# privefl/bigsnpr

Hardware: NVIDIA H100
Metric: genotypes/sec in bed_prodVec (higher is better)
Workload: dtype f64

## Files before the change

### bigsnpr_b200/csrc/bsg_pmv.cu

```cuda
#include <algorithm>
#include <math.h>
#include <stdio.h>
#include <stdlib.h>
#include <string.h>

#include <cub/device/device_scan.cuh>

#include "bsg_internal.cuh"
#include "bsg_pmv_shared.cuh"

namespace bsg {
namespace pmv {

constexpr int SEG = 128;
constexpr int CODES = 512;
constexpr int DIG = 4096;
constexpr int STAGES = 6;
constexpr int STAGE_BYTES = 2 * DIG;
constexpr int SMEM_BYTES = STAGES * STAGE_BYTES + 128;
constexpr int MAX_CHUNKS_PER_ITEM = 512;

struct Args {
  const uint8_t *P;
  int64_t stride;
  const int *lines;
  int nlines;
  int nlines_pad;
  int nchunks;
  int chunks_per_split;
  int ksplit;
  const uint8_t *dig1;
  const uint8_t *dig2;
  const uint8_t *na_flags;
  int use_na;
  long long *part;
};

struct Slot {
  uint4 alo, ahi, blo, bhi;
};

__device__ __forceinline__ void slot_load(Slot &s, const uint8_t *pa, const uint8_t *pb, int64_t off) {
  s.alo = ldg_stream(pa + off);
  s.ahi = ldg_stream(pa + off + 64);
  s.blo = ldg_stream(pb + off);
  s.bhi = ldg_stream(pb + off + 64);
}

template <int MODE>
__device__ __forceinline__ uint32_t plane2(uint32_t x) {
  return MODE == 3 ? (x >> 1) : (x & (x >> 1));
}

template <int MODE, bool PRE>
__device__ __forceinline__ void chunk_mma(const Slot &t0, const Slot &t1, uint32_t dig_addr, int (&acc1)[2][4],
                                          int (&acc16)[2][4], int (&accn1)[2][4], int (&accn16)[2][4]) {
  const uint32_t wA0[8] = {t0.alo.x, t0.alo.y, t0.alo.z, t0.alo.w, t0.ahi.x, t0.ahi.y, t0.ahi.z, t0.ahi.w};
  const uint32_t wB0[8] = {t0.blo.x, t0.blo.y, t0.blo.z, t0.blo.w, t0.bhi.x, t0.bhi.y, t0.bhi.z, t0.bhi.w};
  const uint32_t wA1[8] = {t1.alo.x, t1.alo.y, t1.alo.z, t1.alo.w, t1.ahi.x, t1.ahi.y, t1.ahi.z, t1.ahi.w};
  const uint32_t wB1[8] = {t1.blo.x, t1.blo.y, t1.blo.z, t1.blo.w, t1.bhi.x, t1.bhi.y, t1.bhi.z, t1.bhi.w};
  uint4 dpre[8];
  if (PRE) {
#pragma unroll
    for (int w = 0; w < 8; w++) dpre[w] = lds128(dig_addr + w * 512);
  }
#pragma unroll
  for (int w = 0; w < 8; w++) {
    const uint4 d = PRE ? dpre[w] : lds128(dig_addr + w * 512);
    const uint32_t a0 = wA0[w], b0 = wB0[w], a1 = wA1[w], b1 = wB1[w];
    const uint32_t a0t = a0 >> 2, b0t = b0 >> 2, a1t = a1 >> 2, b1t = b1 >> 2;
    mma_u8s8(acc1[0], a0 & 0x03030303u, b0 & 0x03030303u, a0t & 0x03030303u, b0t & 0x03030303u, d.x, d.y);
    mma_u8s8(acc1[1], a1 & 0x03030303u, b1 & 0x03030303u, a1t & 0x03030303u, b1t & 0x03030303u, d.x, d.y);
    mma_u8s8(acc16[0], a0 & 0x30303030u, b0 & 0x30303030u, a0t & 0x30303030u, b0t & 0x30303030u, d.z, d.w);
    mma_u8s8(acc16[1], a1 & 0x30303030u, b1 & 0x30303030u, a1t & 0x30303030u, b1t & 0x30303030u, d.z, d.w);
    if (MODE != 0) {
      uint4 dn = d;
      if (MODE >= 2) dn = lds128(dig_addr + DIG + w * 512);
      const uint32_t a0n = plane2<MODE>(a0), b0n = plane2<MODE>(b0), a0nt = plane2<MODE>(a0t), b0nt = plane2<MODE>(b0t);
      const uint32_t a1n = plane2<MODE>(a1), b1n = plane2<MODE>(b1), a1nt = plane2<MODE>(a1t), b1nt = plane2<MODE>(b1t);
      mma_u8s8(accn1[0], a0n & 0x01010101u, b0n & 0x01010101u, a0nt & 0x01010101u, b0nt & 0x01010101u, dn.x, dn.y);
      mma_u8s8(accn1[1], a1n & 0x01010101u, b1n & 0x01010101u, a1nt & 0x01010101u, b1nt & 0x01010101u, dn.x, dn.y);
      mma_u8s8(accn16[0], a0n & 0x10101010u, b0n & 0x10101010u, a0nt & 0x10101010u, b0nt & 0x10101010u, dn.z, dn.w);
      mma_u8s8(accn16[1], a1n & 0x10101010u, b1n & 0x10101010u, a1nt & 0x10101010u, b1nt & 0x10101010u, dn.z, dn.w);
    }
  }
}

template <int MODE>
__device__ __forceinline__ void tile_mma(const Slot &sl, const uint4 (&b1)[8], uint32_t dig2_addr, int (&acc1)[4],
                                         int (&acc16)[4], int (&accn1)[4], int (&accn16)[4]) {
  const uint32_t wA[8] = {sl.alo.x, sl.alo.y, sl.alo.z, sl.alo.w, sl.ahi.x, sl.ahi.y, sl.ahi.z, sl.ahi.w};
  const uint32_t wB[8] = {sl.blo.x, sl.blo.y, sl.blo.z, sl.blo.w, sl.bhi.x, sl.bhi.y, sl.bhi.z, sl.bhi.w};
#pragma unroll
  for (int w = 0; w < 8; w++) {
    const uint32_t a = wA[w], bq = wB[w];
    const uint32_t at = a >> 2, bt = bq >> 2;
    mma_u8s8(acc1, a & 0x03030303u, bq & 0x03030303u, at & 0x03030303u, bt & 0x03030303u, b1[w].x, b1[w].y);
    mma_u8s8(acc16, a & 0x30303030u, bq & 0x30303030u, at & 0x30303030u, bt & 0x30303030u, b1[w].z, b1[w].w);
    if (MODE != 0) {
      uint4 d = b1[w];
      if (MODE >= 2) d = lds128(dig2_addr + w * 512);
      const uint32_t an = plane2<MODE>(a), bn = plane2<MODE>(bq);
      const uint32_t ant = plane2<MODE>(at), bnt = plane2<MODE>(bt);
      mma_u8s8(accn1, an & 0x01010101u, bn & 0x01010101u, ant & 0x01010101u, bnt & 0x01010101u, d.x, d.y);
      mma_u8s8(accn16, an & 0x10101010u, bn & 0x10101010u, ant & 0x10101010u, bnt & 0x10101010u, d.z, d.w);
    }
  }
}

template <int MODE, int CW, int R, int STRUCT>
__global__ void __launch_bounds__((CW + 1) * 32, 1) k_pmv(const Args a) {
  constexpr int GROUP = CW * 32;
  extern __shared__ __align__(128) uint8_t smem[];
  const int warp = threadIdx.x >> 5, lane = threadIdx.x & 31;
  const uint32_t smem_base = smem_u32(smem);
  const uint32_t bar_base = smem_base + STAGES * STAGE_BYTES;

  if (threadIdx.x == 0) {
    for (int s = 0; s < STAGES; s++) {
      mbar_init(bar_base + 8 * s, 1);
      mbar_init(bar_base + 8 * (STAGES + s), CW);
    }
    asm volatile("fence.mbarrier_init.release.cluster;" ::: "memory");
  }
  __syncthreads();

  const int ngroups = a.nlines_pad / GROUP;
  const int nitems = ngroups * a.ksplit;
  constexpr bool two_dig = MODE >= 2;
  const uint32_t stage_tx = DIG + (two_dig ? DIG : 0);

  int stage = 0;
  uint32_t phase = 0;

  if (warp == CW) {
    if (lane == 0) {
      for (int item = blockIdx.x; item < nitems; item += gridDim.x) {
        const int group = item / a.ksplit, ks = item - group * a.ksplit;
        const int c0 = ks * a.chunks_per_split;
        const int c1 = min(a.nchunks, c0 + a.chunks_per_split);
        for (int c = c0; c < c1; c++) {
          const uint32_t full = bar_base + 8 * stage, empty = bar_base + 8 * (STAGES + stage);
          mbar_wait(empty, phase ^ 1);
          mbar_expect_tx(full, stage_tx);
          const uint32_t dst = smem_base + stage * STAGE_BYTES;
          bulk_g2s(dst, a.dig1 + (int64_t)c * DIG, DIG, full);
          if (two_dig) bulk_g2s(dst + DIG, a.dig2 + (int64_t)c * DIG, DIG, full);
          if (++stage == STAGES) {
            stage = 0;
            phase ^= 1;
          }
        }
      }
    }
  } else {
    const int g = lane >> 2, q = lane & 3;
    for (int item = blockIdx.x; item < nitems; item += gridDim.x) {
      const int group = item / a.ksplit, ks = item - group * a.ksplit;
      const int c0 = ks * a.chunks_per_split;
      const int c1 = min(a.nchunks, c0 + a.chunks_per_split);
      const uint8_t *pA[2], *pB[2];
#pragma unroll
      for (int u = 0; u < 2; u++) {
        int la = min(group * GROUP + warp * 32 + u * 16 + g, a.nlines - 1);
        int lb = min(group * GROUP + warp * 32 + u * 16 + g + 8, a.nlines - 1);
        const int pa = a.lines ? a.lines[la] : la, pb = a.lines ? a.lines[lb] : lb;
        pA[u] = a.P + (int64_t)pa * a.stride + 16 * q;
        pB[u] = a.P + (int64_t)pb * a.stride + 16 * q;
      }
      bool tile_na = false;
      if (MODE == 3) {
        tile_na = true;
      } else if (MODE != 0) {
        if (a.na_flags) {
          int l = min(group * GROUP + warp * 32 + lane, a.nlines - 1);
          const int phys = a.lines ? a.lines[l] : l;
          tile_na = __any_sync(0xffffffffu, a.na_flags[phys] != 0);
        } else {
          tile_na = true;
        }
      }
      int acc1[2][4], acc16[2][4], accn1[2][4], accn16[2][4];
#pragma unroll
      for (int u = 0; u < 2; u++)
#pragma unroll
        for (int k = 0; k < 4; k++) acc1[u][k] = acc16[u][k] = accn1[u][k] = accn16[u][k] = 0;

      Slot ring[R][2];
#pragma unroll
      for (int k = 0; k < R; k++) {
        ring[k][0] = ring[k][1] =
            Slot{make_uint4(0, 0, 0, 0), make_uint4(0, 0, 0, 0), make_uint4(0, 0, 0, 0), make_uint4(0, 0, 0, 0)};
        if (c0 + k < c1) {
          slot_load(ring[k][0], pA[0], pB[0], (int64_t)(c0 + k) * SEG);
          slot_load(ring[k][1], pA[1], pB[1], (int64_t)(c0 + k) * SEG);
        }
      }

      for (int c = c0; c < c1; c += R) {
#pragma unroll
        for (int par = 0; par < R; par++) {
          if (par > 0 && c + par >= c1) break;
          const uint32_t full = bar_base + 8 * stage, empty = bar_base + 8 * (STAGES + stage);
          mbar_wait(full, phase);
          const uint32_t dbase = smem_base + stage * STAGE_BYTES + (g * 4 + q) * 16;
          const int64_t next = (int64_t)(c + par + R) * SEG;
          const bool more = (c + par + R) < c1;
          if (STRUCT == 0) {
            uint4 b1[8];
#pragma unroll
            for (int w = 0; w < 8; w++) b1[w] = lds128(dbase + w * 512);
#pragma unroll
            for (int u = 0; u < 2; u++) {
              if (MODE != 0 && tile_na)
                tile_mma<MODE>(ring[par][u], b1, dbase + DIG, acc1[u], acc16[u], accn1[u], accn16[u]);
              else
                tile_mma<0>(ring[par][u], b1, 0, acc1[u], acc16[u], accn1[u], accn16[u]);
              if (more) slot_load(ring[par][u], pA[u], pB[u], next);
            }
          } else {
            if (MODE != 0 && tile_na)
              chunk_mma<MODE, STRUCT == 2>(ring[par][0], ring[par][1], dbase, acc1, acc16, accn1, accn16);
            else
              chunk_mma<0, STRUCT == 2>(ring[par][0], ring[par][1], dbase, acc1, acc16, accn1, accn16);
            if (more) {
              slot_load(ring[par][0], pA[0], pB[0], next);
              slot_load(ring[par][1], pA[1], pB[1], next);
            }
          }
          __syncwarp();
          if (lane == 0) mbar_arrive(empty);
          if (++stage == STAGES) {
            stage = 0;
            phase ^= 1;
          }
        }
      }
#pragma unroll
      for (int u = 0; u < 2; u++) {
#pragma unroll
        for (int hrow = 0; hrow < 2; hrow++) {
          const int row = group * GROUP + warp * 32 + u * 16 + g + 8 * hrow;
          unsigned long long *dst = reinterpret_cast<unsigned long long *>(a.part) + (int64_t)row * 16 + 2 * q;
          long long vx = (long long)acc1[u][2 * hrow] + (long long)(acc16[u][2 * hrow] >> 4);
          long long vy = (long long)acc1[u][2 * hrow + 1] + (long long)(acc16[u][2 * hrow + 1] >> 4);
          atomicAdd(dst, (unsigned long long)vx);
          atomicAdd(dst + 1, (unsigned long long)vy);
          if (MODE != 0) {
            long long nx = (long long)accn1[u][2 * hrow] + (long long)(accn16[u][2 * hrow] >> 4);
            long long ny = (long long)accn1[u][2 * hrow + 1] + (long long)(accn16[u][2 * hrow + 1] >> 4);
            atomicAdd(dst + 8, (unsigned long long)nx);
            atomicAdd(dst + 9, (unsigned long long)ny);
          }
        }
      }
    }
  }
}


__device__ __forceinline__ void make_vals(int mode, const double *x, const double *center, const double *scale, int k,
                                          double &v0, double &v1) {
  if (mode == 0) {
    v0 = x[k];
    v1 = 0;
  } else if (mode == 2) {
    v0 = x[k];
    v1 = center[k];
  } else {
    double z = x[k] / scale[k];
    v0 = z;
    v1 = (center[k] - 3.0) * z;
  }
}

__global__ void k_prep1(int mode, const double *__restrict__ x, const double *__restrict__ center,
                        const double *__restrict__ scale, int len, int hb, Scal *sc) {
  __shared__ double sh[32];
  double m0 = 0, m1 = 0, cz = 0;
  int bad = 0;
  for (int k = blockIdx.x * blockDim.x + threadIdx.x; k < len; k += gridDim.x * blockDim.x) {
    double v0, v1;
    make_vals(mode, x, center, scale, k, v0, v1);
    if (!isfinite(v0) || !isfinite(v1)) bad = 1;
    m0 = fmax(m0, fabs(v0));
    m1 = fmax(m1, fabs(v1));
    if (mode == 1) cz += center[k] * v0;
  }
#pragma unroll
  for (int o = 16; o; o >>= 1) {
    m0 = fmax(m0, __shfl_xor_sync(0xffffffffu, m0, o));
    m1 = fmax(m1, __shfl_xor_sync(0xffffffffu, m1, o));
    bad |= __shfl_xor_sync(0xffffffffu, bad, o);
    cz += __shfl_xor_sync(0xffffffffu, cz, o);
  }
  if ((threadIdx.x & 31) == 0) {
    atomicMax(reinterpret_cast<unsigned long long *>(&sc->maxabs[0]), (unsigned long long)__double_as_longlong(m0));
    atomicMax(reinterpret_cast<unsigned long long *>(&sc->maxabs[1]), (unsigned long long)__double_as_longlong(m1));
    if (bad) atomicOr(&sc->nonfinite, 1);
    sh[threadIdx.x >> 5] = cz;
  }
  __syncthreads();
  if (threadIdx.x == 0) {
    double t = 0;
    for (int w = 0; w < (int)(blockDim.x >> 5); w++) t += sh[w];
    sc->cpart[blockIdx.x] = t;
    if (blockIdx.x == 0) sc->hb = hb;
  }
}

__global__ void k_quantise(int mode, const double *__restrict__ x, const double *__restrict__ center,
                           const double *__restrict__ scale, int len, const int *__restrict__ idx, const Scal *sc, int bits,
                           long long *__restrict__ Q0, long long *__restrict__ Q1) {
  const int e0 = pick_e(sc->maxabs[0], sc->hb, bits), e1 = pick_e(sc->maxabs[1], sc->hb, bits);
  const bool bad = sc->nonfinite != 0;
  for (int k = blockIdx.x * blockDim.x + threadIdx.x; k < len; k += gridDim.x * blockDim.x) {
    double v0, v1;
    make_vals(mode, x, center, scale, k, v0, v1);
    const long long q0 = bad ? 0 : __double2ll_rn(scalbn(v0, e0));
    const int t = idx ? idx[k] : k;
    atomicAdd(reinterpret_cast<unsigned long long *>(Q0 + t), (unsigned long long)q0);
    if (Q1) {
      const long long q1 = bad ? 0 : __double2ll_rn(scalbn(v1, e1));
      atomicAdd(reinterpret_cast<unsigned long long *>(Q1 + t), (unsigned long long)q1);
    }
  }
}

template <int NV>
__global__ void k_prep2(int mode, const double *__restrict__ x, const double *__restrict__ center,
                        const double *__restrict__ scale, const double *__restrict__ xb, int len, int nchunks, Scal *sc,
                        const long long *__restrict__ Q0, const long long *__restrict__ Q1, uint8_t *__restrict__ dig1,
                        uint8_t *__restrict__ dig2, int want_sum, long long *__restrict__ qout) {
  constexpr int NS = 8 / NV, BITS = NV == 1 ? 60 : 30;
  const Scal &sa = sc[0], &sb = sc[NV - 1];
  const int ea = pick_e(sa.maxabs[0], sa.hb, BITS), eb = pick_e(sb.maxabs[NV == 1 ? 1 : 0], sb.hb, BITS);
  const bool bada = sa.nonfinite != 0, badb = sb.nonfinite != 0;
  if (blockIdx.x == 0 && threadIdx.x == 0) {
    for (int v = 0; v < NV; v++) {
      sc[v].e[0] = pick_e(sc[v].maxabs[0], sc[v].hb, BITS);
      sc[v].e[1] = pick_e(sc[v].maxabs[1], sc[v].hb, BITS);
    }
  }
  long long hi = 0, lo = 0;
  const bool fasta = ea > -1000 && ea < 1000, fastb = eb > -1000 && eb < 1000;
  const double fa = fasta ? scalbn(1.0, ea) : 0.0, fb = fastb ? scalbn(1.0, eb) : 0.0;
  int64_t total = (int64_t)nchunks * 32;
  for (int64_t t = blockIdx.x * (int64_t)blockDim.x + threadIdx.x; t < total; t += (int64_t)gridDim.x * blockDim.x) {
    const int chunk = (int)(t >> 5), wq = (int)(t & 31);
    const int q = wq & 3, w = wq >> 2;
    uint32_t o1[8][4], o2[8][4];
#pragma unroll
    for (int sl = 0; sl < 8; sl++)
#pragma unroll
      for (int c = 0; c < 4; c++) o1[sl][c] = o2[sl][c] = 0;
#pragma unroll
    for (int c = 0; c < 4; c++) {
#pragma unroll
      for (int r = 0; r < 4; r++) {
        int64_t k = (int64_t)chunk * CODES + (w < 4 ? 64 * q + 16 * w : 256 + 64 * q + 16 * (w - 4)) + 4 * r + c;
        long long qa = 0, qb = 0;
        if (k < len) {
          if (Q0) {
            qa = Q0[k];
            if (Q1) qb = Q1[k];
          } else {
            double v0, v1;
            if (!bada) {
              make_vals(mode, x, center, scale, (int)k, v0, v1);
              qa = __double2ll_rn(fasta ? v0 * fa : scalbn(v0, ea));
              if (NV == 1 && dig2) qb = __double2ll_rn(fastb ? v1 * fb : scalbn(v1, eb));
            }
            if (NV == 2 && xb && !badb) {
              make_vals(mode, xb, center, scale, (int)k, v0, v1);
              qb = __double2ll_rn(fastb ? v0 * fb : scalbn(v0, eb));
            }
          }
        }
        if (want_sum) {
          hi += qa >> 32;
          lo += (long long)(unsigned int)(qa & 0xFFFFFFFFll);
        }
        if (qout && k < len) qout[k] = qa;
#pragma unroll
        for (int sl = 0; sl < NS; sl++) {
          o1[sl][c] |= (uint32_t)(peel(qa) & 0xFF) << (8 * r);
          if (NV == 2)
            o1[NS + sl][c] |= (uint32_t)(peel(qb) & 0xFF) << (8 * r);
          else if (dig2)
            o2[sl][c] |= (uint32_t)(peel(qb) & 0xFF) << (8 * r);
        }
      }
    }
#pragma unroll
    for (int sl = 0; sl < 8; sl++) {
      const int64_t unit = (int64_t)chunk * 256 + (w * 8 + sl) * 4 + q;
      reinterpret_cast<uint4 *>(dig1)[unit] = make_uint4(o1[sl][0], o1[sl][1], o1[sl][2], o1[sl][3]);
      if (NV == 1 && dig2) reinterpret_cast<uint4 *>(dig2)[unit] = make_uint4(o2[sl][0], o2[sl][1], o2[sl][2], o2[sl][3]);
    }
  }
  if (want_sum) {
#pragma unroll
    for (int o = 16; o; o >>= 1) {
      hi += __shfl_xor_sync(0xffffffffu, hi, o);
      lo += __shfl_xor_sync(0xffffffffu, lo, o);
    }
    if ((threadIdx.x & 31) == 0 && (hi | lo)) {
      atomicAdd(reinterpret_cast<unsigned long long *>(&sc->sum_hi), (unsigned long long)hi);
      atomicAdd(reinterpret_cast<unsigned long long *>(&sc->sum_lo), (unsigned long long)lo);
    }
  }
}

__global__ void k_finish_cprod(const long long *__restrict__ part, int nlines, const Scal *sc,
                               const double *__restrict__ center, const double *__restrict__ scale, int use_na,
                               double *__restrict__ out) {
  int j = blockIdx.x * blockDim.x + threadIdx.x;
  if (j >= nlines) return;
  if (sc->nonfinite) {
    out[j] = nan("");
    return;
  }
  const int e = sc->e[0];
  double G = combine<8>(part, j, 0, 1, use_na ? -3 : 0, e);
  double N = use_na ? combine<8>(part, j, 0, 0, 1, e) : 0.0;
  if (center) {
    const double Y = scalbn((double)sc->sum_hi, 32 - e) + scalbn((double)sc->sum_lo, -e);
    out[j] = (G - center[j] * (Y - N)) / scale[j];
  } else {
    out[j] = G;
  }
}

__global__ void k_finish_prod(const long long *__restrict__ part, int nlines, const Scal *sc, int has_scaling, int use_na,
                              double *__restrict__ full) {
  int l = blockIdx.x * blockDim.x + threadIdx.x;
  if (l >= nlines) return;
  full[l] = finish_prod_value(part, l, sc, has_scaling, use_na);
}

__global__ void k_finish_planes(const long long *__restrict__ part, int nlines, const Scal *sc, int have_p, int p_same,
                                double cR, double cP, double add0, double *__restrict__ full, double cRb, double cPb,
                                double *__restrict__ fullB) {
  int l = blockIdx.x * blockDim.x + threadIdx.x;
  if (l >= nlines) return;
  if (sc->nonfinite) {
    full[l] = nan("");
    if (fullB) fullB[l] = nan("");
    return;
  }
  const double R = combine<8>(part, l, 0, 1, 0, sc->e[0]);
  const double P = have_p ? combine<8>(part, l, 0, 0, 1, sc->e[p_same ? 0 : 1]) : 0.0;
  full[l] = (cR * R + cP * P) + add0;
  if (fullB) fullB[l] = cRb * R + cPb * P;
}

__global__ void k_gather(const double *__restrict__ full, const int *__restrict__ idx, int len, double *__restrict__ out) {
  int i = blockIdx.x * blockDim.x + threadIdx.x;
  if (i < len) out[i] = full[idx[i]];
}

constexpr int EV_POOL = 128;
static cudaEvent_t g_ev0[EV_POOL], g_ev1[EV_POOL];
static bool g_ev_ready = false;
static bool g_timing = false;
static int g_ev_n = 0;

static int launch_cap(int64_t work, int block, int cap) {
  int64_t g = (work + block - 1) / block;
  if (g < 1) g = 1;
  if (g > cap) g = cap;
  return (int)g;
}

static int launch_cap_pub_impl(int64_t work) { return launch_cap(work, 256, 132 * 16); }

static int hb_bits(int maxmult) {
  int b = 0;
  while ((1 << b) < maxmult) b++;
  return b >= 8 ? b + 1 : b;
}

static int prep_pmv(bsg_view *v, int dir, int mode, const double *x, const double *p1, const double *p2, int nv,
                    const double *xb, bool two, bool want_sum, bool keep_q, cudaStream_t s) {
  bsg_bed *h = v->h;
  const bool cols = dir == 0;
  const int L = cols ? h->m : h->n, len = cols ? v->nc : v->nr;
  const int *idx = (cols ? v->col_identity : v->row_identity) ? nullptr : (cols ? v->d_col : v->d_row);
  const int hb = hb_bits(cols ? v->col_maxmult : v->row_maxmult);
  const int nchunks = (int)((cols ? h->strideB : h->strideA) / SEG);
  Scal *sc = v->s_scal.as<Scal>();
  BSG_TRY(v->s_dig1.ensure((size_t)nchunks * DIG));
  if (two) BSG_TRY(v->s_dig2.ensure((size_t)nchunks * DIG));
  uint8_t *dig1 = v->s_dig1.as<uint8_t>(), *dig2 = two ? v->s_dig2.as<uint8_t>() : nullptr;
  long long *Q0 = nullptr, *Q1 = nullptr;
  if (idx || keep_q) {
    BSG_TRY(v->s_q0.ensure((size_t)L * sizeof(long long)));
    Q0 = v->s_q0.as<long long>();
  }
  if (idx && (two || xb)) {
    BSG_TRY(v->s_q1.ensure((size_t)L * sizeof(long long)));
    Q1 = v->s_q1.as<long long>();
  }
  BSG_CUDA(cudaMemsetAsync(sc, 0, nv * sizeof(Scal), s));
  k_prep1<<<SUMCZ_BLOCKS, 256, 0, s>>>(mode, x, p1, p2, len, hb, sc);
  if (xb) k_prep1<<<SUMCZ_BLOCKS, 256, 0, s>>>(mode, xb, p1, p2, len, hb, sc + 1);
  count_launch(xb ? 2 : 1);
  if (idx) {
    const int bits = nv == 1 ? 60 : 30;
    BSG_CUDA(cudaMemsetAsync(Q0, 0, (size_t)L * sizeof(long long), s));
    if (Q1) BSG_CUDA(cudaMemsetAsync(Q1, 0, (size_t)L * sizeof(long long), s));
    k_quantise<<<launch_cap(len, 256, 592), 256, 0, s>>>(mode, x, p1, p2, len, idx, sc, bits, Q0, nv == 1 ? Q1 : nullptr);
    if (xb) k_quantise<<<launch_cap(len, 256, 592), 256, 0, s>>>(mode, xb, p1, p2, len, idx, sc + 1, bits, Q1, nullptr);
    count_launch(xb ? 2 : 1);
  }
  const int grid = launch_cap((int64_t)nchunks * 32, 128, 1184);
  const long long *src0 = idx ? Q0 : nullptr;
  if (nv == 1)
    k_prep2<1><<<grid, 128, 0, s>>>(mode, x, p1, p2, nullptr, L, nchunks, sc, src0, Q1, dig1, dig2, want_sum,
                                    idx ? nullptr : Q0);
  else
    k_prep2<2><<<grid, 128, 0, s>>>(mode, x, p1, p2, xb, L, nchunks, sc, src0, Q1, dig1, nullptr, want_sum, nullptr);
  count_launch();
  return BSG_OK;
}

static int run_pmv(bsg_view *v, const uint8_t *P, int64_t stride, int L, const int *lines, int nlines,
                   const uint8_t *dig1, const uint8_t *dig2, const uint8_t *na_flags, int use_na, Args *out_args,
                   cudaStream_t s, bool plane_hi = false) {
  static int var_cw = 0, var_r = 0, var_s = 0;
  if (!var_cw) {
    var_cw = 11;
    var_r = 3;
    var_s = 1;
    const char *ev = getenv("BSG_PMV_VARIANT");
    int cw = 0, r = 0, st = 0;
    if (ev && sscanf(ev, "%dx%ds%d", &cw, &r, &st) >= 2) {
      if ((cw == 11 || cw == 15) && (r == 2 || r == 3) && st >= 0 && st <= 2) {
        var_cw = cw;
        var_r = r;
        var_s = st;
      }
    }
  }
  const int GROUP = var_cw * 32;
  Args a;
  a.P = P;
  a.stride = stride;
  a.lines = lines;
  a.nlines = nlines;
  a.nlines_pad = (int)round_up(nlines, GROUP);
  a.nchunks = (int)(round_up(((int64_t)L + 3) / 4, SEG) / SEG);
  int ngroups = a.nlines_pad / GROUP;
  int target_items = 24 * 132;
  int ks = (target_items + ngroups - 1) / ngroups;
  int ks_max = std::max(1, a.nchunks / 16);
  int ks_min = (a.nchunks + MAX_CHUNKS_PER_ITEM - 1) / MAX_CHUNKS_PER_ITEM;
  ks = std::min(ks, ks_max);
  ks = std::max(ks, ks_min);
  ks = std::max(ks, 1);
  a.chunks_per_split = (a.nchunks + ks - 1) / ks;
  a.ksplit = (a.nchunks + a.chunks_per_split - 1) / a.chunks_per_split;
  a.dig1 = dig1;
  a.dig2 = dig2;
  a.na_flags = na_flags;
  a.use_na = use_na;
  BSG_TRY(v->s_part.ensure((size_t)a.nlines_pad * 16 * sizeof(long long)));
  a.part = v->s_part.as<long long>();
  BSG_CUDA(cudaMemsetAsync(a.part, 0, (size_t)a.nlines_pad * 16 * sizeof(long long), s));
  const int mode = plane_hi ? 3 : (!use_na ? 0 : (dig2 ? 2 : 1));
  if (plane_hi && !dig2) return fail(BSG_ERR_ARG, "high-bit plane needs its own digits");
  void (*kern)(const Args) = nullptr;
#define PMV_PICK(CWv, Rv, Sv)                                                                   \
  if (var_cw == CWv && var_r == Rv && var_s == Sv)                                              \
    kern = mode == 0 ? k_pmv<0, CWv, Rv, Sv>                                                    \
                     : (mode == 1 ? k_pmv<1, CWv, Rv, Sv> : (mode == 2 ? k_pmv<2, CWv, Rv, Sv> : k_pmv<3, CWv, Rv, Sv>));
  PMV_PICK(11, 2, 0)
  PMV_PICK(11, 2, 1)
  PMV_PICK(11, 2, 2)
  PMV_PICK(11, 3, 0)
  PMV_PICK(11, 3, 1)
  PMV_PICK(15, 2, 1)
#undef PMV_PICK
  if (!kern) return fail(BSG_ERR_ARG, "unknown k_pmv variant");
  BSG_CUDA(cudaFuncSetAttribute(kern, cudaFuncAttributeMaxDynamicSharedMemorySize, SMEM_BYTES));
  int nsm = 132;
  cudaDeviceGetAttribute(&nsm, cudaDevAttrMultiProcessorCount, v->h->device);
  int nitems = ngroups * a.ksplit;
  int grid = std::min(nitems, nsm);
  if (g_timing) cudaEventRecord(g_ev0[g_ev_n % EV_POOL], s);
  kern<<<grid, (var_cw + 1) * 32, SMEM_BYTES, s>>>(a);
  if (g_timing) {
    cudaEventRecord(g_ev1[g_ev_n % EV_POOL], s);
    g_ev_n++;
  }
  count_launch();
  BSG_CUDA(cudaGetLastError());
  *out_args = a;
  return BSG_OK;
}

}

namespace pmvt {
using namespace pmv;
constexpr int TLINES = 32, TBYTES = 512, TWARPS = 8, TSTAGES = 6;
constexpr int WSTAGE_BYTES = TLINES * 64;
constexpr int TSMEM = TWARPS * TSTAGES * WSTAGE_BYTES;
constexpr int MAX_LINES_PER_ITEM = 1 << 16;

struct TArgs {
  const uint8_t *P;
  int64_t stride;
  const int *lines;
  int nlines;
  const uint8_t *dig;
  int lines_per_split, ksplit, nblocks, n;
  long long *part;
};

__device__ __forceinline__ void cp_async16(uint32_t dst, const void *src, int src_bytes) {
  asm volatile("cp.async.cg.shared.global [%0], [%1], 16, %2;" ::"r"(dst), "l"(src), "r"(src_bytes) : "memory");
}

template <int PLANE>
__global__ void __launch_bounds__(TWARPS * 32, 2) k_pmvT_lines(const TArgs a) {
  extern __shared__ __align__(128) uint8_t smem[];
  const int tid = threadIdx.x, warp = tid >> 5, lane = tid & 31, g = lane >> 2, q = lane & 3;
  const int blk = blockIdx.x % a.nblocks, ks = blockIdx.x / a.nblocks;
  const int64_t byte0 = (int64_t)blk * TBYTES + 64 * warp;
  const int l0 = ks * a.lines_per_split, l1 = min(a.nlines, l0 + a.lines_per_split);
  const int nsteps = (l1 - l0 + TLINES - 1) / TLINES;
  const uint32_t wbase = smem_u32(smem) + warp * (TSTAGES * WSTAGE_BYTES);

  const int lrow = lane >> 2, lch = lane & 3;
  const int64_t colb = (byte0 + 16 * lch < a.stride) ? byte0 + 16 * lch : 0;
  uint32_t dst_off[4];
#pragma unroll
  for (int i = 0; i < 4; i++) {
    const int row = 8 * i + lrow;
    const int hf = row >> 4, qq = (row >> 2) & 3, r = row & 3, sl = lch >> 1, hc = lch & 1;
    dst_off[i] = (uint32_t)((((((r * 2 + hf) * 2 + sl) * 4 + qq) * 8) + 4 * hc) * 4);
  }
  auto issue = [&](int step, int stage) {
    const uint32_t dst = wbase + stage * WSTAGE_BYTES;
#pragma unroll
    for (int i = 0; i < 4; i++) {
      const int t = min(l0 + step * TLINES + 8 * i + lrow, l1 - 1);
      const int phys = a.lines[t];
      cp_async16(dst + dst_off[i], a.P + colb + (int64_t)phys * a.stride, 16);
    }
  };

  int acc[4][4][4];
#pragma unroll
  for (int j = 0; j < 4; j++)
#pragma unroll
    for (int c = 0; c < 4; c++)
#pragma unroll
      for (int k = 0; k < 4; k++) acc[j][c][k] = 0;

#pragma unroll
  for (int st = 0; st < TSTAGES - 1; st++) {
    if (st < nsteps) issue(st, st);
    asm volatile("cp.async.commit_group;" ::: "memory");
  }
  const uint8_t *dg = a.dig + (int64_t)(l0 / TLINES) * 256 + g * 32 + 4 * q;
  uint32_t nb0 = 0, nb1 = 0;
  if (nsteps > 0) {
    nb0 = *reinterpret_cast<const uint32_t *>(dg);
    nb1 = *reinterpret_cast<const uint32_t *>(dg + 16);
  }
  const uint32_t rd_base = wbase + (uint32_t)((q * 8 + g) * 4);

  auto compute = [&](uint32_t st_base, uint32_t b0, uint32_t b1) {
    uint32_t W[2][2][4];
#pragma unroll
    for (int sl = 0; sl < 2; sl++)
#pragma unroll
      for (int hf = 0; hf < 2; hf++) {
        const uint32_t ad = st_base + (hf * 2 + sl) * 128;
        const uint32_t x0 = lds32(ad), x1 = lds32(ad + 512), x2 = lds32(ad + 1024), x3 = lds32(ad + 1536);
        const uint32_t t0 = prmt(x0, x1, 0x5140), t1 = prmt(x2, x3, 0x5140);
        const uint32_t t2 = prmt(x0, x1, 0x7362), t3 = prmt(x2, x3, 0x7362);
        W[sl][hf][0] = prmt(t0, t1, 0x5410);
        W[sl][hf][1] = prmt(t0, t1, 0x7632);
        W[sl][hf][2] = prmt(t2, t3, 0x5410);
        W[sl][hf][3] = prmt(t2, t3, 0x7632);
      }
#pragma unroll
    for (int j = 0; j < 4; j++) {
      uint32_t wa = W[0][0][j], wb = W[1][0][j], wc2 = W[0][1][j], wd = W[1][1][j];
      if (PLANE == 1) {
        wa = wa & (wa >> 1) & 0x55555555u;
        wb = wb & (wb >> 1) & 0x55555555u;
        wc2 = wc2 & (wc2 >> 1) & 0x55555555u;
        wd = wd & (wd >> 1) & 0x55555555u;
      } else if (PLANE == 2) {
        wa = (wa >> 1) & 0x55555555u;
        wb = (wb >> 1) & 0x55555555u;
        wc2 = (wc2 >> 1) & 0x55555555u;
        wd = (wd >> 1) & 0x55555555u;
      }
      mma_u8s8(acc[j][0], wa & 0x03030303u, wb & 0x03030303u, wc2 & 0x03030303u, wd & 0x03030303u, b0, b1);
      mma_u8s8(acc[j][1], wa & 0x0C0C0C0Cu, wb & 0x0C0C0C0Cu, wc2 & 0x0C0C0C0Cu, wd & 0x0C0C0C0Cu, b0, b1);
      mma_u8s8(acc[j][2], wa & 0x30303030u, wb & 0x30303030u, wc2 & 0x30303030u, wd & 0x30303030u, b0, b1);
      mma_u8s8(acc[j][3], wa & 0xC0C0C0C0u, wb & 0xC0C0C0C0u, wc2 & 0xC0C0C0C0u, wd & 0xC0C0C0C0u, b0, b1);
    }
  };

  uint32_t rd_stage = 0, wr_stage = (TSTAGES - 1) * WSTAGE_BYTES;
  const uint8_t *dgn = dg + 256;
  for (int step = 0; step < nsteps; step++) {
    asm volatile("cp.async.wait_group %0;" ::"n"(TSTAGES - 2) : "memory");
    __syncwarp();
    {
      const int nxt = step + TSTAGES - 1;
      if (nxt < nsteps) issue(nxt, (int)(wr_stage / WSTAGE_BYTES));
      asm volatile("cp.async.commit_group;" ::: "memory");
    }
    const uint32_t b0 = nb0, b1 = nb1;
    if (step + 1 < nsteps) {
      nb0 = *reinterpret_cast<const uint32_t *>(dgn);
      nb1 = *reinterpret_cast<const uint32_t *>(dgn + 16);
      dgn += 256;
    }
    compute(rd_base + rd_stage, b0, b1);
    rd_stage = rd_stage + WSTAGE_BYTES == TSTAGES * WSTAGE_BYTES ? 0 : rd_stage + WSTAGE_BYTES;
    wr_stage = wr_stage + WSTAGE_BYTES == TSTAGES * WSTAGE_BYTES ? 0 : wr_stage + WSTAGE_BYTES;
  }
  asm volatile("cp.async.wait_group 0;" ::: "memory");
#pragma unroll
  for (int j = 0; j < 4; j++)
#pragma unroll
    for (int c = 0; c < 4; c++)
#pragma unroll
      for (int sl = 0; sl < 2; sl++) {
        const int64_t sample = 4 * (byte0 + 4 * (8 * sl + g) + j) + c;
        if (sample < a.n) {
          unsigned long long *dst = reinterpret_cast<unsigned long long *>(a.part) + sample * 16 + (PLANE ? 8 : 0) + 2 * q;
          long long v0 = acc[j][c][2 * sl], v1 = acc[j][c][2 * sl + 1];
          v0 >>= 2 * c;
          v1 >>= 2 * c;
          if (v0) atomicAdd(dst, (unsigned long long)v0);
          if (v1) atomicAdd(dst + 1, (unsigned long long)v1);
        }
      }
}

constexpr int TBOX = 32 * 128;
constexpr int TDIG_OFF = 4 * TBOX;
constexpr int TSTAGE_BYTES = 4 * TBOX + 1024;
constexpr int TCSTAGES = 6;
constexpr int TSMEM_TMA = TCSTAGES * TSTAGE_BYTES + 2 * TCSTAGES * 8 + 1024;


template <int PLANE>
__global__ void __launch_bounds__(TWARPS * 32, 2) k_pmvT(const __grid_constant__ CUtensorMap map, const TArgs a) {
  extern __shared__ __align__(128) uint8_t smem[];
  const int tid = threadIdx.x, warp = tid >> 5, lane = tid & 31, g = lane >> 2, q = lane & 3;
  const int blk = blockIdx.x % a.nblocks, ks = blockIdx.x / a.nblocks;
  const int l0 = ks * a.lines_per_split, l1 = min(a.nlines, l0 + a.lines_per_split);
  const int nsteps = (l1 - l0 + TLINES - 1) / TLINES;
  const uint32_t sbase = (smem_u32(smem) + 1023u) & ~1023u;
  const uint32_t bar_base = sbase + TCSTAGES * TSTAGE_BYTES;
  auto fill = [&](int step, int st) {
    const uint32_t full = bar_base + 8 * st, dst = sbase + st * TSTAGE_BYTES;
    const uint8_t *dg = a.dig + (int64_t)(l0 / TLINES + step) * 256;
    mbar_expect_tx(full, 4 * TBOX + 256);
#pragma unroll
    for (int j = 0; j < 4; j++) tma_load_2d(dst + j * TBOX, &map, full, blk * TBYTES + 128 * j, l0 + step * TLINES);
    bulk_g2s(dst + TDIG_OFF, dg, 128, full);
    bulk_g2s(dst + TDIG_OFF + 144, dg + 128, 128, full);
  };
  if (tid == 0) {
    for (int st = 0; st < TCSTAGES; st++) {
      mbar_init(bar_base + 8 * st, 1);
      mbar_init(bar_base + 8 * (TCSTAGES + st), TWARPS);
    }
    asm volatile("fence.mbarrier_init.release.cluster;" ::: "memory");
    for (int st = 0; st < min(TCSTAGES, nsteps); st++) fill(st, st);
  }
  __syncthreads();
  int stage = 0, pstage = 0;
  uint32_t phase = 0, pphase = 0;

  const int64_t byte0 = (int64_t)blk * TBYTES + 64 * warp;
  const int rsw = 2 * (q >> 1);
  const uint32_t chunk0 = (4 * (warp & 1) + (g >> 2)) ^ (4 * (q & 1) + rsw);
  const uint32_t rd_base = sbase + (warp >> 1) * TBOX + q * 512 + (rsw << 7) + chunk0 * 16 + 4 * (g & 3);
  const uint32_t dg_base = sbase + TDIG_OFF + g * 32 + 16 * (g >> 2) + 4 * q;
  const uint32_t sel_lo = rsw ? 0x1054u : 0x5410u, sel_hi = rsw ? 0x3276u : 0x7632u;

  int acc[4][4][4];
#pragma unroll
  for (int j = 0; j < 4; j++)
#pragma unroll
    for (int c = 0; c < 4; c++)
#pragma unroll
      for (int k = 0; k < 4; k++) acc[j][c][k] = 0;

  for (int step = 0; step < nsteps; step++) {
    const uint32_t full = bar_base + 8 * stage, empty = bar_base + 8 * (TCSTAGES + stage);
    const uint32_t so = stage * TSTAGE_BYTES;
    const int cstage = stage;
    const uint32_t cphase = phase;
    mbar_wait(full, phase);
    const uint32_t b0 = lds32(dg_base + so), b1 = lds32(dg_base + so + 16);
    uint32_t W[2][2][4];
#pragma unroll
    for (int sl = 0; sl < 2; sl++)
#pragma unroll
      for (int hf = 0; hf < 2; hf++) {
        const uint32_t ad = rd_base + so, hb = hf * (16 * 128);
        const uint32_t x0 = lds32((ad ^ TRD(0, sl)) + hb), x1 = lds32((ad ^ TRD(1, sl)) + hb);
        const uint32_t x2 = lds32((ad ^ TRD(2, sl)) + hb), x3 = lds32((ad ^ TRD(3, sl)) + hb);
        const uint32_t t0 = prmt(x0, x1, 0x5140), t1 = prmt(x2, x3, 0x5140);
        const uint32_t t2 = prmt(x0, x1, 0x7362), t3 = prmt(x2, x3, 0x7362);
        W[sl][hf][0] = prmt(t0, t1, sel_lo);
        W[sl][hf][1] = prmt(t0, t1, sel_hi);
        W[sl][hf][2] = prmt(t2, t3, sel_lo);
        W[sl][hf][3] = prmt(t2, t3, sel_hi);
      }
    __syncwarp();
    if (lane == 0) mbar_arrive(empty);
    if (++stage == TCSTAGES) {
      stage = 0;
      phase ^= 1;
    }
#pragma unroll
    for (int j = 0; j < 4; j++) {
      uint32_t wa = W[0][0][j], wb = W[1][0][j], wc2 = W[0][1][j], wd = W[1][1][j];
      if (PLANE == 1) {
        wa = wa & (wa >> 1) & 0x55555555u;
        wb = wb & (wb >> 1) & 0x55555555u;
        wc2 = wc2 & (wc2 >> 1) & 0x55555555u;
        wd = wd & (wd >> 1) & 0x55555555u;
      } else if (PLANE == 2) {
        wa = (wa >> 1) & 0x55555555u;
        wb = (wb >> 1) & 0x55555555u;
        wc2 = (wc2 >> 1) & 0x55555555u;
        wd = (wd >> 1) & 0x55555555u;
      }
      mma_u8s8(acc[j][0], wa & 0x03030303u, wb & 0x03030303u, wc2 & 0x03030303u, wd & 0x03030303u, b0, b1);
      mma_u8s8(acc[j][1], wa & 0x0C0C0C0Cu, wb & 0x0C0C0C0Cu, wc2 & 0x0C0C0C0Cu, wd & 0x0C0C0C0Cu, b0, b1);
      mma_u8s8(acc[j][2], wa & 0x30303030u, wb & 0x30303030u, wc2 & 0x30303030u, wd & 0x30303030u, b0, b1);
      mma_u8s8(acc[j][3], wa & 0xC0C0C0C0u, wb & 0xC0C0C0C0u, wc2 & 0xC0C0C0C0u, wd & 0xC0C0C0C0u, b0, b1);
    }
    if (tid == 0 && step >= 1 && step - 1 + TCSTAGES < nsteps) {
      mbar_wait(bar_base + 8 * (TCSTAGES + pstage), pphase);
      fill(step - 1 + TCSTAGES, pstage);
    }
    __syncwarp();
    pstage = cstage;
    pphase = cphase;
  }
#pragma unroll
  for (int j = 0; j < 4; j++)
#pragma unroll
    for (int c = 0; c < 4; c++)
#pragma unroll
      for (int sl = 0; sl < 2; sl++) {
        const int64_t sample = 4 * (byte0 + 4 * (8 * sl + g) + j) + c;
        if (sample < a.n) {
          unsigned long long *dst = reinterpret_cast<unsigned long long *>(a.part) + sample * 16 + (PLANE ? 8 : 0) + 2 * q;
          long long v0 = acc[j][c][2 * sl], v1 = acc[j][c][2 * sl + 1];
          v0 >>= 2 * c;
          v1 >>= 2 * c;
          if (v0) atomicAdd(dst, (unsigned long long)v0);
          if (v1) atomicAdd(dst + 1, (unsigned long long)v1);
        }
      }
}

constexpr int W2STAGE_BYTES = TLINES * 32;
constexpr int T2BYTES = TWARPS * 32;
constexpr int T2SMEM = TWARPS * TSTAGES * W2STAGE_BYTES;

template <int PL, bool LINES>
__global__ void __launch_bounds__(TWARPS * 32, 2) k_pmvT2(const TArgs a, const uint8_t *__restrict__ dig2) {
  extern __shared__ __align__(128) uint8_t smem[];
  const int tid = threadIdx.x, warp = tid >> 5, lane = tid & 31, g = lane >> 2, q = lane & 3;
  const int blk = blockIdx.x % a.nblocks, ks = blockIdx.x / a.nblocks;
  const int64_t byte0 = (int64_t)blk * T2BYTES + 32 * warp;
  const int l0 = ks * a.lines_per_split, l1 = min(a.nlines, l0 + a.lines_per_split);
  const int nsteps = (l1 - l0 + TLINES - 1) / TLINES;
  const uint32_t wbase = smem_u32(smem) + warp * (TSTAGES * W2STAGE_BYTES);
  const int lrow = lane >> 1, lch = lane & 1;
  const int64_t colb = (byte0 + 16 * lch < a.stride) ? byte0 + 16 * lch : 0;
  uint32_t dst_off[2];
#pragma unroll
  for (int i = 0; i < 2; i++) {
    const int row = 16 * i + lrow;
    const int hf = row >> 4, qq = (row >> 2) & 3, r = row & 3;
// ... 1292 lines not shown
```

Baseline: 11640 billion.

## Add warp-specialized staged PMV kernel with bulk-async smem pipeline as default

Adds k_pmvs, a new kernel in which four producer warps issue per-row bulk global-to-shared copies (plus digit planes) into a multi-stage mbarrier ring sized to fill the opt-in shared memory. Eight consumer warps split chunks across K and run the existing MMA path from padded shared rows, with a pitch chosen to avoid bank conflicts. Run_pmv now defaults to this staged path, with smaller groups, fewer target items, and chunks_per_split rounded to the chunks-per-stage count. The intent is to better hide memory latency and raise bandwidth utilisation. In exchange it uses a very large smem footprint at one block per SM, and many small per-row bulk copies could add overhead.

```diff
diff --git a/bigsnpr_b200/csrc/bsg_pmv.cu b/bigsnpr_b200/csrc/bsg_pmv.cu
--- a/bigsnpr_b200/csrc/bsg_pmv.cu
+++ b/bigsnpr_b200/csrc/bsg_pmv.cu
@@ -241,6 +241,159 @@
 #pragma unroll
         for (int hrow = 0; hrow < 2; hrow++) {
           const int row = group * GROUP + warp * 32 + u * 16 + g + 8 * hrow;
+          unsigned long long *dst = reinterpret_cast<unsigned long long *>(a.part) + (int64_t)row * 16 + 2 * q;
+          long long vx = (long long)acc1[u][2 * hrow] + (long long)(acc16[u][2 * hrow] >> 4);
+          long long vy = (long long)acc1[u][2 * hrow + 1] + (long long)(acc16[u][2 * hrow + 1] >> 4);
+          atomicAdd(dst, (unsigned long long)vx);
+          atomicAdd(dst + 1, (unsigned long long)vy);
+          if (MODE != 0) {
+            long long nx = (long long)accn1[u][2 * hrow] + (long long)(accn16[u][2 * hrow] >> 4);
+            long long ny = (long long)accn1[u][2 * hrow + 1] + (long long)(accn16[u][2 * hrow + 1] >> 4);
+            atomicAdd(dst + 8, (unsigned long long)nx);
+            atomicAdd(dst + 9, (unsigned long long)ny);
+          }
+        }
+      }
+    }
+  }
+}
+
+constexpr int SW = 8;
+constexpr int SP = 4;
+constexpr int SMEM_OPTIN = 227 * 1024;
+template <int MODE, int LW, int CPS>
+struct Staged {
+  static constexpr int GROUP = 32 * LW, KW = SW / LW, PITCH = CPS * SEG + 64;
+  static constexpr int DPITCH = MODE >= 2 ? 2 * DIG : DIG;
+  static constexpr int STAGE = GROUP * PITCH + CPS * DPITCH;
+  static constexpr int NST = (SMEM_OPTIN - 256) / STAGE;
+  static constexpr int SMEM = NST * STAGE + 16 * NST;
+  static_assert(SW % LW == 0 && LW % SP == 0 && CPS % KW == 0 && NST >= 2 && MAX_CHUNKS_PER_ITEM % CPS == 0,
+                "staged geometry");
+  static_assert(PITCH % 128 == 64, "fragment rows g and g + 1 must fall on opposite halves of the 128-byte bank line");
+};
+constexpr int STAGED_LW = 4, STAGED_CPS = 4;
+
+template <int MODE, int LW, int CPS>
+__global__ void __launch_bounds__((SW + SP) * 32, 1) k_pmvs(const Args a) {
+  using K = Staged<MODE, LW, CPS>;
+  extern __shared__ __align__(128) uint8_t smem[];
+  const int warp = threadIdx.x >> 5, lane = threadIdx.x & 31;
+  const uint32_t smem_base = smem_u32(smem);
+  const uint32_t bar_base = smem_base + K::NST * K::STAGE;
+
+  if (threadIdx.x == 0) {
+    for (int s = 0; s < K::NST; s++) {
+      mbar_init(bar_base + 8 * s, 1);
+      mbar_init(bar_base + 8 * (K::NST + s), SW);
+    }
+    asm volatile("fence.mbarrier_init.release.cluster;" ::: "memory");
+  }
+  __syncthreads();
+
+  const int ngroups = a.nlines_pad / K::GROUP;
+  const int nitems = ngroups * a.ksplit;
+  constexpr int planes = MODE >= 2 ? 2 : 1;
+  int stage = 0;
+  uint32_t phase = 0;
+
+  if (warp >= SW) {
+    const int p = warp - SW;
+    for (int item = blockIdx.x; item < nitems; item += gridDim.x) {
+      const int group = item / a.ksplit, ks = item - group * a.ksplit;
+      const int c0 = ks * a.chunks_per_split;
+      const int c1 = min(a.nchunks, c0 + a.chunks_per_split);
+      const uint8_t *src[LW];
+#pragma unroll
+      for (int i = 0; i < LW; i++) {
+        if (i % SP != p) continue;
+        const int l = min(group * K::GROUP + 32 * i + lane, a.nlines - 1);
+        src[i] = a.P + (int64_t)(a.lines ? a.lines[l] : l) * a.stride;
+      }
+      for (int c = c0; c < c1; c += CPS) {
+        const int nv = min(CPS, c1 - c);
+        const uint32_t full = bar_base + 8 * stage, empty = bar_base + 8 * (K::NST + stage);
+        const uint32_t dst = smem_base + stage * K::STAGE;
+        mbar_wait(empty, phase ^ 1);
+        if (p == 0 && lane == 0) mbar_expect_tx(full, nv * (K::GROUP * SEG + planes * DIG));
+        __syncwarp();
+#pragma unroll
+        for (int i = 0; i < LW; i++)
+          if (i % SP == p) bulk_g2s(dst + (32 * i + lane) * K::PITCH, src[i] + (int64_t)c * SEG, nv * SEG, full);
+        if (p == 0 && lane < planes * nv) {
+          const int j = lane % nv, pl = lane / nv;
+          bulk_g2s(dst + K::GROUP * K::PITCH + j * K::DPITCH + pl * DIG, (pl ? a.dig2 : a.dig1) + (int64_t)(c + j) * DIG,
+                   DIG, full);
+        }
+        if (++stage == K::NST) {
+          stage = 0;
+          phase ^= 1;
+        }
+      }
+    }
+  } else {
+    const int lt = warp % LW, kc = warp / LW;
+    const int g = lane >> 2, q = lane & 3;
+    for (int item = blockIdx.x; item < nitems; item += gridDim.x) {
+      const int group = item / a.ksplit, ks = item - group * a.ksplit;
+      const int c0 = ks * a.chunks_per_split;
+      const int c1 = min(a.nchunks, c0 + a.chunks_per_split);
+      bool tile_na = false;
+      if (MODE == 3) {
+        tile_na = true;
+      } else if (MODE != 0) {
+        if (a.na_flags) {
+          int l = min(group * K::GROUP + lt * 32 + lane, a.nlines - 1);
+          const int phys = a.lines ? a.lines[l] : l;
+          tile_na = __any_sync(0xffffffffu, a.na_flags[phys] != 0);
+        } else {
+          tile_na = true;
+        }
+      }
+      int acc1[2][4], acc16[2][4], accn1[2][4], accn16[2][4];
+#pragma unroll
+      for (int u = 0; u < 2; u++)
+#pragma unroll
+        for (int k = 0; k < 4; k++) acc1[u][k] = acc16[u][k] = accn1[u][k] = accn16[u][k] = 0;
+
+      for (int c = c0; c < c1; c += CPS) {
+        const int nv = min(CPS, c1 - c);
+        const uint32_t full = bar_base + 8 * stage, empty = bar_base + 8 * (K::NST + stage);
+        const uint32_t st = smem_base + stage * K::STAGE;
+        const uint32_t rows = st + (lt * 32 + g) * K::PITCH + 16 * q;
+        const uint32_t dig = st + K::GROUP * K::PITCH + (g * 4 + q) * 16;
+        mbar_wait(full, phase);
+#pragma unroll
+        for (int j0 = 0; j0 < CPS; j0 += K::KW) {
+          const int j = j0 + kc;
+          if (j < nv) {
+            Slot t[2];
+#pragma unroll
+            for (int u = 0; u < 2; u++) {
+              const uint32_t r = rows + u * 16 * K::PITCH + j * SEG;
+              t[u].alo = lds128(r);
+              t[u].ahi = lds128(r + 64);
+              t[u].blo = lds128(r + 8 * K::PITCH);
+              t[u].bhi = lds128(r + 8 * K::PITCH + 64);
+            }
+            if (MODE != 0 && tile_na)
+              chunk_mma<MODE, false>(t[0], t[1], dig + j * K::DPITCH, acc1, acc16, accn1, accn16);
+            else
+              chunk_mma<0, false>(t[0], t[1], dig + j * K::DPITCH, acc1, acc16, accn1, accn16);
+          }
+        }
+        __syncwarp();
+        if (lane == 0) mbar_arrive(empty);
+        if (++stage == K::NST) {
+          stage = 0;
+          phase ^= 1;
+        }
+      }
+#pragma unroll
+      for (int u = 0; u < 2; u++) {
+#pragma unroll
+        for (int hrow = 0; hrow < 2; hrow++) {
+          const int row = group * K::GROUP + lt * 32 + u * 16 + g + 8 * hrow;
           unsigned long long *dst = reinterpret_cast<unsigned long long *>(a.part) + (int64_t)row * 16 + 2 * q;
           long long vx = (long long)acc1[u][2 * hrow] + (long long)(acc16[u][2 * hrow] >> 4);
           long long vy = (long long)acc1[u][2 * hrow + 1] + (long long)(acc16[u][2 * hrow + 1] >> 4);
@@ -528,11 +681,9 @@
 static int run_pmv(bsg_view *v, const uint8_t *P, int64_t stride, int L, const int *lines, int nlines,
                    const uint8_t *dig1, const uint8_t *dig2, const uint8_t *na_flags, int use_na, Args *out_args,
                    cudaStream_t s, bool plane_hi = false) {
-  static int var_cw = 0, var_r = 0, var_s = 0;
-  if (!var_cw) {
-    var_cw = 11;
-    var_r = 3;
-    var_s = 1;
+  static int var_cw = -1, var_r = 0, var_s = 0;
+  if (var_cw < 0) {
+    var_cw = 0;
     const char *ev = getenv("BSG_PMV_VARIANT");
     int cw = 0, r = 0, st = 0;
     if (ev && sscanf(ev, "%dx%ds%d", &cw, &r, &st) >= 2) {
@@ -543,7 +694,8 @@
       }
     }
   }
-  const int GROUP = var_cw * 32;
+  const bool staged = var_cw == 0;
+  const int GROUP = staged ? 32 * STAGED_LW : var_cw * 32;
   Args a;
   a.P = P;
   a.stride = stride;
@@ -552,7 +704,7 @@
   a.nlines_pad = (int)round_up(nlines, GROUP);
   a.nchunks = (int)(round_up(((int64_t)L + 3) / 4, SEG) / SEG);
   int ngroups = a.nlines_pad / GROUP;
-  int target_items = 24 * 132;
+  int target_items = (staged ? 4 : 24) * 132;
   int ks = (target_items + ngroups - 1) / ngroups;
   int ks_max = std::max(1, a.nchunks / 16);
   int ks_min = (a.nchunks + MAX_CHUNKS_PER_ITEM - 1) / MAX_CHUNKS_PER_ITEM;
@@ -560,6 +712,7 @@
   ks = std::max(ks, ks_min);
   ks = std::max(ks, 1);
   a.chunks_per_split = (a.nchunks + ks - 1) / ks;
+  if (staged) a.chunks_per_split = (int)round_up(a.chunks_per_split, STAGED_CPS);
   a.ksplit = (a.nchunks + a.chunks_per_split - 1) / a.chunks_per_split;
   a.dig1 = dig1;
   a.dig2 = dig2;
@@ -571,6 +724,14 @@
   const int mode = plane_hi ? 3 : (!use_na ? 0 : (dig2 ? 2 : 1));
   if (plane_hi && !dig2) return fail(BSG_ERR_ARG, "high-bit plane needs its own digits");
   void (*kern)(const Args) = nullptr;
+  int smem = SMEM_BYTES, block = (var_cw + 1) * 32;
+  if (staged) {
+    constexpr int LW = STAGED_LW, CPS = STAGED_CPS;
+    kern = mode == 0 ? k_pmvs<0, LW, CPS>
+                     : (mode == 1 ? k_pmvs<1, LW, CPS> : (mode == 2 ? k_pmvs<2, LW, CPS> : k_pmvs<3, LW, CPS>));
+    smem = mode >= 2 ? Staged<2, LW, CPS>::SMEM : Staged<0, LW, CPS>::SMEM;
+    block = (SW + SP) * 32;
+  }
 #define PMV_PICK(CWv, Rv, Sv)                                                                   \
   if (var_cw == CWv && var_r == Rv && var_s == Sv)                                              \
     kern = mode == 0 ? k_pmv<0, CWv, Rv, Sv>                                                    \
@@ -583,13 +744,13 @@
   PMV_PICK(15, 2, 1)
 #undef PMV_PICK
   if (!kern) return fail(BSG_ERR_ARG, "unknown k_pmv variant");
-  BSG_CUDA(cudaFuncSetAttribute(kern, cudaFuncAttributeMaxDynamicSharedMemorySize, SMEM_BYTES));
+  BSG_CUDA(cudaFuncSetAttribute(kern, cudaFuncAttributeMaxDynamicSharedMemorySize, smem));
   int nsm = 132;
   cudaDeviceGetAttribute(&nsm, cudaDevAttrMultiProcessorCount, v->h->device);
   int nitems = ngroups * a.ksplit;
   int grid = std::min(nitems, nsm);
   if (g_timing) cudaEventRecord(g_ev0[g_ev_n % EV_POOL], s);
-  kern<<<grid, (var_cw + 1) * 32, SMEM_BYTES, s>>>(a);
+  kern<<<grid, block, smem, s>>>(a);
   if (g_timing) {
     cudaEventRecord(g_ev1[g_ev_n % EV_POOL], s);
     g_ev_n++;
```

After: 11640 billion (median of 6 runs). Within noise of the previous version (+0.0%).
